# AuburnSounds/audio-formats

Measured on AMD Instinct MI355X. Metric: decoded samples/sec (batched MP3+OGG+FLAC) at 1/2/4/8 MI355X vs CPU ref, higher is better.
Workload: dtype f32 (MP3, Vorbis, CELT) + int32 (FLAC)

## Files before the change

### audio-formats_amd/csrc/mp3_kernel.h

```cpp
#pragma once
#include "afg_common.h"
#ifndef AFG_MP3_FMA
#error "define AFG_MP3_FMA (0 / 1) and AFG_MP3_KERNEL before including mp3_kernel.h"
#endif

#ifndef AFG_MP3_NT_LOAD
#define AFG_MP3_NT_LOAD 0
#endif
#if AFG_MP3_NT_LOAD
typedef float afg_f32x2 __attribute__((ext_vector_type(2)));
#define AFG_MP3_LD(p) ([&] { const afg_f32x2 t_ = __builtin_nontemporal_load((const afg_f32x2 *)(p)); return f2{ t_.x, t_.y }; }())
#else
#define AFG_MP3_LD(p) (*(p))
#endif
#ifndef AFG_MP3_NT_STORE
#define AFG_MP3_NT_STORE 1
#endif

namespace {

struct Mp3Seg {
    uint32_t stream;
    uint32_t g0;
    uint32_t count;
    uint32_t last;
};

struct Mp3Stream {
    uint64_t blk_base;
    uint32_t ngr;
    uint32_t nch;
};

constexpr int kStateOverlap = 64 * 9;

__device__ const float k_aa_cs[8] = {
    0.85749293f, 0.88174200f, 0.94962865f, 0.98331459f, 0.99551782f, 0.99916056f, 0.99989920f, 0.99999316f };
__device__ const float k_aa_ca[8] = {
    0.51449576f, 0.47173197f, 0.31337745f, 0.18191320f, 0.09457419f, 0.04096558f, 0.01419856f, 0.00369997f };

__device__ const float k_win[15 * 16] = {
    -1, 26, -31, 208, 218, 401, -519, 2063, 2000, 4788, -5517, 7134, 5959, 35640, -39336, 74992,
    -1, 24, -35, 202, 222, 347, -581, 2080, 1952, 4425, -5879, 7640, 5288, 33791, -41176, 74856,
    -1, 21, -38, 196, 225, 294, -645, 2087, 1893, 4063, -6237, 8092, 4561, 31947, -43006, 74630,
    -1, 19, -41, 190, 227, 244, -711, 2085, 1822, 3705, -6589, 8492, 3776, 30112, -44821, 74313,
    -1, 17, -45, 183, 228, 197, -779, 2075, 1739, 3351, -6935, 8840, 2935, 28289, -46617, 73908,
    -1, 16, -49, 176, 228, 153, -848, 2057, 1644, 3004, -7271, 9139, 2037, 26482, -48390, 73415,
    -2, 14, -53, 169, 227, 111, -919, 2032, 1535, 2663, -7597, 9389, 1082, 24694, -50137, 72835,
    -2, 13, -58, 161, 224, 72, -991, 2001, 1414, 2330, -7910, 9592, 70, 22929, -51853, 72169,
    -2, 11, -63, 154, 221, 36, -1064, 1962, 1280, 2006, -8209, 9750, -998, 21189, -53534, 71420,
    -2, 10, -68, 147, 215, 2, -1137, 1919, 1131, 1692, -8491, 9863, -2122, 19478, -55178, 70590,
    -3, 9, -73, 139, 208, -29, -1210, 1870, 970, 1388, -8755, 9935, -3300, 17799, -56778, 69679,
    -3, 8, -79, 132, 200, -57, -1283, 1817, 794, 1095, -8998, 9966, -4533, 16155, -58333, 68692,
    -4, 7, -85, 125, 189, -83, -1356, 1759, 605, 814, -9219, 9959, -5818, 14548, -59838, 67629,
    -4, 7, -91, 117, 177, -106, -1428, 1698, 402, 545, -9416, 9916, -7154, 12980, -61289, 66494,
    -5, 6, -97, 111, 163, -127, -1498, 1634, 185, 288, -9585, 9838, -8540, 11455, -62684, 65290 };

__device__ __forceinline__ void dct3_9(float (&y)[9])
{
    float e0 = y[0], e2 = y[2], e4 = y[4], e6 = y[6], e8 = y[8];
    float m0 = e0 + e6 * 0.5f;
    e0 = e0 - e6;
    float m4 = (e4 + e2) * 0.93969262f;
    float m2 = (e8 + e2) * 0.76604444f;
    e6 = (e4 - e8) * 0.17364818f;
    e4 = e4 + (e8 - e2);

    e2 = e0 - e4 * 0.5f;
    y[4] = e4 + e0;
    e8 = m0 - m2 + e6;
    e0 = m0 - m4 + m2;
    e4 = m0 + m4 - e6;

    float o1 = y[1], o3 = y[3], o5 = y[5], o7 = y[7];
    o3 = o3 * 0.86602540f;
    m0 = (o5 + o1) * 0.98480775f;
    m4 = (o5 - o7) * 0.34202014f;
    m2 = (o1 + o7) * 0.64278761f;
    o1 = (o1 - o5 - o7) * 0.86602540f;

    o5 = m0 - o3 - m2;
    o7 = m4 - o3 - m0;
    o3 = m4 + o3 - m2;

    y[0] = e4 - o7;
    y[1] = e2 + o1;
    y[2] = e0 - o3;
    y[3] = e8 + o5;
    y[5] = e8 - o5;
    y[6] = e0 + o3;
    y[7] = e2 - o1;
    y[8] = e4 + o7;
}

__device__ __forceinline__ void imdct36_lane(float (&x)[18], float (&ov)[9], bool stop)
{
    constexpr float tw[18] = {
        0.73727734f, 0.79335334f, 0.84339145f, 0.88701083f, 0.92387953f, 0.95371695f, 0.97629601f, 0.99144486f, 0.99904822f,
        0.67559021f, 0.60876143f, 0.53729961f, 0.46174861f, 0.38268343f, 0.30070580f, 0.21643961f, 0.13052619f, 0.04361938f };
    constexpr float w0[18] = {
        0.99904822f, 0.99144486f, 0.97629601f, 0.95371695f, 0.92387953f, 0.88701083f, 0.84339145f, 0.79335334f, 0.73727734f,
        0.04361938f, 0.13052619f, 0.21643961f, 0.30070580f, 0.38268343f, 0.46174861f, 0.53729961f, 0.60876143f, 0.67559021f };
    constexpr float w1[18] = {
        1, 1, 1, 1, 1, 1, 0.99144486f, 0.92387953f, 0.79335334f,
        0, 0, 0, 0, 0, 0, 0.13052619f, 0.38268343f, 0.60876143f };

    float co[9], si[9];
    co[0] = -x[0];
    si[0] = x[17];
#pragma unroll
    for (int i = 0; i < 4; i++) {
        si[8 - 2 * i] = x[4 * i + 1] - x[4 * i + 2];
        co[1 + 2 * i] = x[4 * i + 1] + x[4 * i + 2];
        si[7 - 2 * i] = x[4 * i + 4] - x[4 * i + 3];
        co[2 + 2 * i] = -(x[4 * i + 3] + x[4 * i + 4]);
    }
    dct3_9(co);
    dct3_9(si);
    si[1] = -si[1];
    si[3] = -si[3];
    si[5] = -si[5];
    si[7] = -si[7];
#pragma unroll
    for (int i = 0; i < 9; i++) {
        float wa = stop ? w1[i] : w0[i];
        float wb = stop ? w1[9 + i] : w0[9 + i];
        float ovl = ov[i];
        float sum = co[i] * tw[9 + i] + si[i] * tw[i];
        ov[i] = co[i] * tw[i] - si[i] * tw[9 + i];
        x[i] = ovl * wa - sum * wb;
        x[17 - i] = ovl * wb + sum * wa;
    }
}

__device__ __forceinline__ void idct3(float x0, float x1, float x2, float (&dst)[3])
{
    float m1 = x1 * 0.86602540f;
    float a1 = x0 - x2 * 0.5f;
    dst[1] = x0 + x2;
    dst[0] = a1 + m1;
    dst[2] = a1 - m1;
}

__device__ __forceinline__ void imdct12(const float (&t)[18], int off, float (&dst)[6], float (&ov)[3])
{
    constexpr float tw3[6] = { 0.79335334f, 0.92387953f, 0.99144486f, 0.60876143f, 0.38268343f, 0.13052619f };
    float co[3], si[3];
    idct3(-t[off + 0], t[off + 6] + t[off + 3], t[off + 12] + t[off + 9], co);
    idct3(t[off + 15], t[off + 12] - t[off + 9], t[off + 6] - t[off + 3], si);
    si[1] = -si[1];
#pragma unroll
    for (int i = 0; i < 3; i++) {
        float ovl = ov[i];
        float sum = co[i] * tw3[3 + i] + si[i] * tw3[i];
        ov[i] = co[i] * tw3[i] - si[i] * tw3[3 + i];
        dst[i] = ovl * tw3[2 - i] - sum * tw3[5 - i];
        dst[5 - i] = ovl * tw3[5 - i] + sum * tw3[2 - i];
    }
}

__device__ __forceinline__ void imdct_short_lane(float (&x)[18], float (&ov)[9])
{
    float t[18];
#pragma unroll
    for (int i = 0; i < 18; i++) t[i] = x[i];
#pragma unroll
    for (int i = 0; i < 6; i++) x[i] = ov[i];
    float tail[3] = { ov[6], ov[7], ov[8] };
    float d[6];
    imdct12(t, 0, d, tail);
#pragma unroll
    for (int i = 0; i < 6; i++) x[6 + i] = d[i];
    imdct12(t, 1, d, tail);
#pragma unroll
    for (int i = 0; i < 6; i++) x[12 + i] = d[i];
    imdct12(t, 2, d, tail);
#pragma unroll
    for (int i = 0; i < 6; i++) ov[i] = d[i];
    ov[6] = tail[0];
    ov[7] = tail[1];
    ov[8] = tail[2];
}

__device__ __forceinline__ void dct2_32(const float (&in)[32], float (&out)[32])
{
    constexpr float sec[24] = {
        10.19000816f, 0.50060302f, 0.50241929f, 3.40760851f, 0.50547093f, 0.52249861f, 2.05778098f, 0.51544732f,
        0.56694406f, 1.48416460f, 0.53104258f, 0.64682180f, 1.16943991f, 0.55310392f, 0.78815460f, 0.97256821f,
        0.58293498f, 1.06067765f, 0.83934963f, 0.62250412f, 1.72244716f, 0.74453628f, 0.67480832f, 5.10114861f };
    float t[4][8];
#pragma unroll
    for (int i = 0; i < 8; i++) {
        float x0 = in[i];
        float x1 = in[15 - i];
        float x2 = in[16 + i];
        float x3 = in[31 - i];
        float t0 = x0 + x3;
        float t1 = x1 + x2;
        float t2 = (x1 - x2) * sec[3 * i + 0];
        float t3 = (x0 - x3) * sec[3 * i + 1];
        t[0][i] = t0 + t1;
        t[1][i] = (t0 - t1) * sec[3 * i + 2];
        t[2][i] = t3 + t2;
        t[3][i] = (t3 - t2) * sec[3 * i + 2];
    }
#pragma unroll
    for (int r = 0; r < 4; r++) {
        float x0 = t[r][0], x1 = t[r][1], x2 = t[r][2], x3 = t[r][3];
        float x4 = t[r][4], x5 = t[r][5], x6 = t[r][6], x7 = t[r][7], xt;
        xt = x0 - x7; x0 = x0 + x7;
        x7 = x1 - x6; x1 = x1 + x6;
        x6 = x2 - x5; x2 = x2 + x5;
        x5 = x3 - x4; x3 = x3 + x4;
        x4 = x0 - x3; x0 = x0 + x3;
        x3 = x1 - x2; x1 = x1 + x2;
        t[r][0] = x0 + x1;
        t[r][4] = (x0 - x1) * 0.70710677f;
        x5 = x5 + x6;
        x6 = (x6 + x7) * 0.70710677f;
        x7 = x7 + xt;
        x3 = (x3 + x4) * 0.70710677f;
        x5 = x5 - x7 * 0.198912367f;
        x7 = x7 + x5 * 0.382683432f;
        x5 = x5 - x7 * 0.198912367f;
        x0 = xt - x6; xt = xt + x6;
        t[r][1] = (xt + x7) * 0.50979561f;
        t[r][2] = (x4 + x3) * 0.54119611f;
        t[r][3] = (x0 - x5) * 0.60134488f;
        t[r][5] = (x0 + x5) * 0.89997619f;
        t[r][6] = (x4 - x3) * 1.30656302f;
        t[r][7] = (xt - x7) * 2.56291556f;
    }
#pragma unroll
    for (int i = 0; i < 7; i++) {
        out[4 * i + 0] = t[0][i];
        out[4 * i + 1] = t[2][i] + t[3][i] + t[3][i + 1];
        out[4 * i + 2] = t[1][i] + t[1][i + 1];
        out[4 * i + 3] = t[2][i + 1] + t[3][i] + t[3][i + 1];
    }
    out[28] = t[0][7];
    out[29] = t[2][7] + t[3][7];
    out[30] = t[1][7];
    out[31] = t[3][7];
}

constexpr int kHS = 66;
constexpr int kHistRows = 15;
constexpr int kRegion = kHistRows * kHS;
constexpr int kLdsFloats = 33 * kHS;
constexpr int kWinStride = 18;

struct alignas(8) f2 { float x, y; };

#define WAVE_SYNC() __builtin_amdgcn_wave_barrier()

__device__ __forceinline__ float from_lane_below(float v)
{
    return __int_as_float(__builtin_amdgcn_update_dpp(0, __float_as_int(v), 0x138, 0xf, 0xf, false));
}
__device__ __forceinline__ float from_lane_above(float v)
{
    return __int_as_float(__builtin_amdgcn_update_dpp(0, __float_as_int(v), 0x130, 0xf, 0xf, false));
}

#ifndef AFG_MP3_MIN_WAVES
#define AFG_MP3_MIN_WAVES 4
#endif

template <int NCH>
__device__ __forceinline__ void mp3_segment(
    const Mp3Seg &seg, const Mp3Stream &st, const float *__restrict__ coef, const uint32_t *__restrict__ flags,
    float *__restrict__ pcm, float *__restrict__ state, float *const H, float *const Wt)
{
    float *const R = H + kRegion;
    const int lane = threadIdx.x;
    constexpr int nch = NCH;
    constexpr int nval = nch * 576;

    const int ch = lane >> 5;
    const int band = lane & 31;
    const int s2 = lane >> 5;
    const int sc = (lane >> 4) & 1;
    const int si = lane & 15;

    const f2 *const wrow = (const f2 *)(Wt + (14 - (si < 15 ? si : 14)) * kWinStride);

    float ov[9];
    const int n_warm = seg.g0 < 2u ? (int)seg.g0 : 2;
    const int g_first = (int)seg.g0 - n_warm;
    const bool from_state = (g_first == 0) && (state != nullptr);
    float *st_blob = state ? state + (size_t)seg.stream * AFG_MP3_STATE_FLOATS : nullptr;
#pragma unroll
    for (int i = 0; i < 9; i++) ov[i] = from_state ? st_blob[lane * 9 + i] : 0.0f;
    for (int r = 0; r < kHistRows; r++)
        H[r * kHS + lane] = from_state ? st_blob[kStateOverlap + r * 64 + lane] : 0.0f;

    const int g_end = (int)(seg.g0 + seg.count);
    const bool ch_on = ch < nch;
    int fbase = g_first;
    uint32_t fl_a = 0, fl_b = 0;
    auto refill = [&](int gb) {
        fbase = gb;
        const int gi = gb + lane;
        fl_a = fl_b = 0;
        if (gi < g_end) {
            fl_a = flags[st.blk_base + (uint64_t)gi * nch];
            if (nch == 2) fl_b = flags[st.blk_base + (uint64_t)gi * nch + 1];
        }
        asm volatile("" : "+v"(fl_a), "+v"(fl_b) : : "memory");
    };
    refill(g_first);
    auto loads_of = [&](int g) -> bool {
        const uint32_t w0 = (uint32_t)__builtin_amdgcn_readlane((int)fl_a, g - fbase);
        const uint32_t w1 = (uint32_t)__builtin_amdgcn_readlane((int)fl_b, g - fbase);
        const uint32_t nz = ((ch ? w1 : w0) >> 24) & 63u;
        return ch_on && band < (int)(nz ? nz - 1u : 32u);
    };
    f2 pre[9];
    {
        const f2 *src = (const f2 *)(coef + (st.blk_base + (uint64_t)g_first * nch) * 576) + lane * 9;
        const bool on = loads_of(g_first);
#pragma unroll
        for (int q = 0; q < 9; q++) pre[q] = f2{ 0.0f, 0.0f };
        if (on) {
#pragma unroll
            for (int q = 0; q < 9; q++) pre[q] = AFG_MP3_LD(src + q);
        }
    }
#pragma unroll
    for (int q = 0; q < 9; q++) asm volatile("" : "+v"(pre[q].x), "+v"(pre[q].y) : : "memory");
    WAVE_SYNC();

    for (int g = g_first; g < g_end; g++) {
        const bool do_synth = g >= (int)seg.g0;
        const bool do_dct = g >= (int)seg.g0 - 1;

        float x[18];
#pragma unroll
        for (int m = 0; m < 9; m++) {
            x[2 * m] = pre[m].x;
            x[2 * m + 1] = pre[m].y;
        }
        if (g + 1 - fbase >= 64) refill(g);
        const uint32_t fl0 = (uint32_t)__builtin_amdgcn_readlane((int)fl_a, g - fbase);
        const uint32_t fl1 = (uint32_t)__builtin_amdgcn_readlane((int)fl_b, g - fbase);
        const uint32_t fl = ch_on ? (ch ? fl1 : fl0) : 0u;
        if (g + 1 < g_end) {
            const f2 *src = (const f2 *)(coef + (st.blk_base + (uint64_t)(g + 1) * nch) * 576) + lane * 9;
            const bool on = loads_of(g + 1);
#pragma unroll
            for (int q = 0; q < 9; q++) pre[q] = f2{ 0.0f, 0.0f };
            if (on) {
#pragma unroll
                for (int q = 0; q < 9; q++) pre[q] = AFG_MP3_LD(src + q);
            }
        }

        if (!(fl0 >> 31)) {
            const int block_type = (int)(fl & 3u);
            const int n_long = (int)((fl >> 8) & 0xffu);
            const int aa = (int)((fl >> 16) & 0xffu) - 1;
            const bool lower = (band >= 1) && (band - 1 < aa);
            const bool upper = (band < aa);
            float nl[8], nh[8];
#pragma unroll
            for (int i = 0; i < 8; i++) {
                float d_prev = from_lane_below(x[17 - i]);
                float u_next = from_lane_above(x[i]);
                nl[i] = x[i] * k_aa_cs[i] - d_prev * k_aa_ca[i];
                nh[i] = u_next * k_aa_ca[i] + x[17 - i] * k_aa_cs[i];
            }
#pragma unroll
            for (int i = 0; i < 8; i++) {
                x[i] = lower ? nl[i] : x[i];
                x[17 - i] = upper ? nh[i] : x[17 - i];
            }
            const bool is_short = (block_type == 2) && (band >= n_long);
            if (is_short) {
                imdct_short_lane(x, ov);
            } else {
                const bool stop = (block_type == 3) && (band >= n_long);
                imdct36_lane(x, ov, stop);
            }
            if (band & 1) {
#pragma unroll
                for (int i = 1; i < 18; i += 2) x[i] = -x[i];
            }
        }

        if (do_dct) {
#pragma unroll
            for (int m = 0; m < 9; m++) ((f2 *)R)[lane * 9 + m] = f2{ x[2 * m], x[2 * m + 1] };
            WAVE_SYNC();

            float out[32];
            const bool dct_lane = (band < 18) && ch_on;
            {
                float in[32];
                const float *col = R + ch * 576 + (dct_lane ? band : 0);
#pragma unroll
                for (int b = 0; b < 32; b++) in[b] = col[b * 18];
                dct2_32(in, out);
            }
            WAVE_SYNC();
            if (dct_lane) {
                f2 *row = (f2 *)(R + band * kHS + ch * 32);
#pragma unroll
                for (int i = 0; i < 15; i++) row[i] = f2{ out[31 - i], out[1 + i] };
                row[15] = f2{ out[16], out[0] };
            }
            WAVE_SYNC();
        }

        if (do_synth) {
            float op0 = 0.0f, op16 = 0.0f;
            const bool pair_lane = (band < 18) && ch_on;
            if (pair_lane) {
                const f2 *base = (const f2 *)(H + band * kHS + ch * 32) + 15;
                f2 z[15];
#pragma unroll
                for (int m = 0; m < 15; m++) z[m] = base[m * (kHS / 2)];
                float a;
                a  = (z[14].x - z[0].x) * 29;
                a += (z[1].x + z[13].x) * 213;
                a += (z[12].x - z[2].x) * 459;
                a += (z[3].x + z[11].x) * 2037;
                a += (z[10].x - z[4].x) * 5153;
                a += (z[5].x + z[9].x) * 6574;
                a += (z[8].x - z[6].x) * 37489;
                a += z[7].x * 75038;
                op0 = a * (1.0f / 32768.0f);
                a  = z[14].y * 104;
                a += z[12].y * 1567;
                a += z[10].y * 9727;
                a += z[8].y * 64019;
                a += z[6].y * -9975;
                a += z[4].y * -45;
                a += z[2].y * 146;
                a += z[0].y * -5;
                op16 = a * (1.0f / 32768.0f);
            }

            f2 w[8];
#pragma unroll
            for (int k = 0; k < 8; k++) w[k] = wrow[k];
            const bool main_lane = (si < 15) && (sc < nch);
            const f2 *base = (const f2 *)(H + s2 * kHS + sc * 32) + (si < 15 ? si : 14);
            const float *rbase = (const float *)base;
            float rw[32];
#pragma unroll
            for (int m = 0; m < 18; m++) rw[m] = rbase[m * kHS + (((m & 1) ^ 0) ? 0 : 1)];
#pragma unroll
            for (int n = 0; n < 9; n++) {
                if (n + 1 < 9 && n > 0) {
                    rw[16 + 2 * n] = rbase[(16 + 2 * n) * kHS + 1];
                    rw[17 + 2 * n] = rbase[(17 + 2 * n) * kHS + 0];
                }
                float a = 0.0f, b = 0.0f;
#pragma unroll
                for (int k = 0; k < 8; k++) {
                    const float vz = rw[15 + 2 * n - k];
                    const float vy = rw[2 * n + k];
#if AFG_MP3_FMA
                    b = __builtin_fmaf(vz, w[k].y, b);
                    b = __builtin_fmaf(vy, w[k].x, b);
                    if (k & 1) {
                        a = __builtin_fmaf(vy, w[k].y, a);
                        a = __builtin_fmaf(-vz, w[k].x, a);
                    } else {
                        a = __builtin_fmaf(vz, w[k].x, a);
                        a = __builtin_fmaf(-vy, w[k].y, a);
                    }
#else
                    const float tb = vz * w[k].y + vy * w[k].x;
                    const float ta = (k & 1) ? (vy * w[k].y - vz * w[k].x) : (vz * w[k].x - vy * w[k].y);
                    b = (k == 0) ? tb : (b + tb);
                    a = (k == 0) ? ta : (a + ta);
#endif
                }
                if (main_lane) {
                    float *pdst = H + ((2 * n + s2) * 32) * nch + sc;
                    pdst[(15 - si) * nch] = a * (1.0f / 32768.0f);
                    pdst[(17 + si) * nch] = b * (1.0f / 32768.0f);
                }
            }
            if (pair_lane) {
                float *pp = H + (band * 32) * nch + ch;
                pp[0] = op0;
                pp[16 * nch] = op16;
            }
            WAVE_SYNC();
#pragma unroll
            for (int q = 0; q < 9; q++) asm volatile("" : "+v"(pre[q].x), "+v"(pre[q].y) : : "memory");
            float4 *dst = (float4 *)(pcm + (st.blk_base + (uint64_t)g * nch) * 576);
#pragma unroll
            for (int q = 0; q < 5; q++) {
                const int idx = lane + 64 * q;
#if AFG_MP3_NT_STORE
                if (4 * idx < nval) {
                    typedef float f32x4nt __attribute__((ext_vector_type(4)));
                    __builtin_nontemporal_store(((const f32x4nt *)H)[idx], (f32x4nt *)dst + idx);
                }
#else
                if (4 * idx < nval) dst[idx] = ((const float4 *)H)[idx];
#endif
            }
        }
        WAVE_SYNC();

        if (do_dct) {
            constexpr int n2 = kHistRows * kHS / 2;
            const f2 *srcp = (const f2 *)(H + 18 * kHS);
            f2 hcp[8];
#pragma unroll
            for (int q = 0; q < 8; q++) {
                const int idx = lane + 64 * q;
                hcp[q] = (idx < n2) ? srcp[idx] : f2{ 0.0f, 0.0f };
            }
#pragma unroll
            for (int q = 0; q < 8; q++) {
                const int idx = lane + 64 * q;
                if (idx < n2) ((f2 *)H)[idx] = hcp[q];
            }
        }
        WAVE_SYNC();
    }

    if (st_blob && seg.last) {
#pragma unroll
        for (int i = 0; i < 9; i++) st_blob[lane * 9 + i] = ov[i];
        for (int r = 0; r < kHistRows; r++) st_blob[kStateOverlap + r * 64 + lane] = H[r * kHS + lane];
    }
}


__global__ __launch_bounds__(64, AFG_MP3_MIN_WAVES) void AFG_MP3_KERNEL(
    const Mp3Seg *__restrict__ segs, const Mp3Stream *__restrict__ streams,
    const float *__restrict__ coef, const uint32_t *__restrict__ flags,
    float *__restrict__ pcm, float *__restrict__ state)
{
    __shared__ __attribute__((aligned(16))) float H[kLdsFloats];
    __shared__ __attribute__((aligned(16))) float Wt[15 * kWinStride];
    const int lane = threadIdx.x;
    for (int i = lane; i < 15 * 16; i += 64) Wt[(i >> 4) * kWinStride + (i & 15)] = k_win[i];
    const Mp3Seg seg = segs[blockIdx.x];
    const Mp3Stream st = streams[seg.stream];
    if (st.nch == 2) mp3_segment<2>(seg, st, coef, flags, pcm, state, H, Wt);
    else mp3_segment<1>(seg, st, coef, flags, pcm, state, H, Wt);
}

}
```

Measured before the change: 795.5 billion.

## Double-buffer MP3 synthesis history in LDS to drop per-granule history copy

```diff
diff --git a/audio-formats_amd/csrc/mp3_kernel.h b/audio-formats_amd/csrc/mp3_kernel.h
--- a/audio-formats_amd/csrc/mp3_kernel.h
+++ b/audio-formats_amd/csrc/mp3_kernel.h
@@ -244,11 +244,19 @@
     out[31] = t[3][7];
 }
 
+#ifndef AFG_MP3_STAGE_PAD
+#define AFG_MP3_STAGE_PAD 1
+#endif
 constexpr int kHS = 66;
 constexpr int kHistRows = 15;
-constexpr int kRegion = kHistRows * kHS;
-constexpr int kLdsFloats = 33 * kHS;
+constexpr int kHalfRows = 18;
+constexpr int kHalf = kHalfRows * kHS;
+constexpr int kHistRow0 = kHalfRows - kHistRows;
+constexpr int kLdsFloats = (2 * kHalfRows + AFG_MP3_STAGE_PAD) * kHS;
+constexpr int kZLen = 3 * kHalfRows;
 constexpr int kWinStride = 18;
+__host__ __device__ constexpr int kStage(int nch) { return 32 * nch + 4 * AFG_MP3_STAGE_PAD; }
+static_assert(17 * kStage(2) + 64 <= kLdsFloats - kHalf, "the staged PCM of a granule leaves the buffer");
 
 struct alignas(8) f2 { float x, y; };
 
@@ -264,15 +272,14 @@
 }
 
 #ifndef AFG_MP3_MIN_WAVES
-#define AFG_MP3_MIN_WAVES 4
+#define AFG_MP3_MIN_WAVES 3
 #endif
 
 template <int NCH>
 __device__ __forceinline__ void mp3_segment(
     const Mp3Seg &seg, const Mp3Stream &st, const float *__restrict__ coef, const uint32_t *__restrict__ flags,
-    float *__restrict__ pcm, float *__restrict__ state, float *const H, float *const Wt)
-{
-    float *const R = H + kRegion;
+    float *__restrict__ pcm, float *__restrict__ state, float *const H, float *const Z, float *const Wt)
+{
     const int lane = threadIdx.x;
     constexpr int nch = NCH;
     constexpr int nval = nch * 576;
@@ -292,8 +299,14 @@
     float *st_blob = state ? state + (size_t)seg.stream * AFG_MP3_STATE_FLOATS : nullptr;
 #pragma unroll
     for (int i = 0; i < 9; i++) ov[i] = from_state ? st_blob[lane * 9 + i] : 0.0f;
-    for (int r = 0; r < kHistRows; r++)
-        H[r * kHS + lane] = from_state ? st_blob[kStateOverlap + r * 64 + lane] : 0.0f;
+    const bool z_lane = (lane & 31) >= 30;
+    float *const zf = Z + ((lane >> 5) * kZLen) * 2 + (lane & 1);
+    for (int r = 0; r < kHistRows; r++) {
+        const float v = from_state ? st_blob[kStateOverlap + r * 64 + lane] : 0.0f;
+        if (z_lane) zf[(kHistRow0 + r) * 2] = v;
+        else H[(kHistRow0 + r) * kHS + lane] = v;
+    }
+    int phase = 0;
 
     const int g_end = (int)(seg.g0 + seg.count);
     const bool ch_on = ch < nch;
@@ -334,6 +347,8 @@
     for (int g = g_first; g < g_end; g++) {
         const bool do_synth = g >= (int)seg.g0;
         const bool do_dct = g >= (int)seg.g0 - 1;
+        const int ob = phase ? kHalf : 0;
+        const int nb = kHalf - ob;
 
         float x[18];
 #pragma unroll
@@ -390,24 +405,30 @@
 
         if (do_dct) {
 #pragma unroll
-            for (int m = 0; m < 9; m++) ((f2 *)R)[lane * 9 + m] = f2{ x[2 * m], x[2 * m + 1] };
+            for (int m = 0; m < 9; m++) ((f2 *)(H + nb))[lane * 9 + m] = f2{ x[2 * m], x[2 * m + 1] };
             WAVE_SYNC();
 
             float out[32];
             const bool dct_lane = (band < 18) && ch_on;
             {
                 float in[32];
-                const float *col = R + ch * 576 + (dct_lane ? band : 0);
+                const float *col = H + nb + ch * 576 + (dct_lane ? band : 0);
 #pragma unroll
                 for (int b = 0; b < 32; b++) in[b] = col[b * 18];
                 dct2_32(in, out);
             }
             WAVE_SYNC();
             if (dct_lane) {
-                f2 *row = (f2 *)(R + band * kHS + ch * 32);
+                f2 *row = (f2 *)(H + nb + band * kHS + ch * 32);
 #pragma unroll
                 for (int i = 0; i < 15; i++) row[i] = f2{ out[31 - i], out[1 + i] };
-                row[15] = f2{ out[16], out[0] };
+                f2 *zrow = (f2 *)Z + ch * kZLen + band;
+                if (phase) {
+                    zrow[0] = f2{ out[16], out[0] };
+                    zrow[2 * kHalfRows] = f2{ out[16], out[0] };
+                } else {
+                    zrow[kHalfRows] = f2{ out[16], out[0] };
+                }
             }
             WAVE_SYNC();
         }
@@ -416,10 +437,10 @@
             float op0 = 0.0f, op16 = 0.0f;
             const bool pair_lane = (band < 18) && ch_on;
             if (pair_lane) {
-                const f2 *base = (const f2 *)(H + band * kHS + ch * 32) + 15;
+                const f2 *base = (const f2 *)Z + ch * kZLen + band + (phase ? kHalfRows + kHistRow0 : kHistRow0);
                 f2 z[15];
 #pragma unroll
-                for (int m = 0; m < 15; m++) z[m] = base[m * (kHS / 2)];
+                for (int m = 0; m < 15; m++) z[m] = base[m];
                 float a;
                 a  = (z[14].x - z[0].x) * 29;
                 a += (z[1].x + z[13].x) * 213;
@@ -445,16 +466,21 @@
 #pragma unroll
             for (int k = 0; k < 8; k++) w[k] = wrow[k];
             const bool main_lane = (si < 15) && (sc < nch);
-            const f2 *base = (const f2 *)(H + s2 * kHS + sc * 32) + (si < 15 ? si : 14);
-            const float *rbase = (const float *)base;
+            const int wcol = sc * 32 + 2 * (si < 15 ? si : 14);
+            const float *rO = H + ob + (kHistRow0 + s2) * kHS + wcol;
+            const float *rN = H + nb + s2 * kHS + wcol;
+            const float *r14 = s2 ? rN - kHS : rO + 14 * kHS;
             float rw[32];
 #pragma unroll
-            for (int m = 0; m < 18; m++) rw[m] = rbase[m * kHS + (((m & 1) ^ 0) ? 0 : 1)];
+            for (int m = 0; m < 14; m++) rw[m] = rO[m * kHS + ((m & 1) ? 0 : 1)];
+            rw[14] = r14[1];
+#pragma unroll
+            for (int m = 15; m < 18; m++) rw[m] = rN[(m - 15) * kHS + ((m & 1) ? 0 : 1)];
 #pragma unroll
             for (int n = 0; n < 9; n++) {
                 if (n + 1 < 9 && n > 0) {
-                    rw[16 + 2 * n] = rbase[(16 + 2 * n) * kHS + 1];
-                    rw[17 + 2 * n] = rbase[(17 + 2 * n) * kHS + 0];
+                    rw[16 + 2 * n] = rN[(1 + 2 * n) * kHS + 1];
+                    rw[17 + 2 * n] = rN[(2 + 2 * n) * kHS + 0];
                 }
                 float a = 0.0f, b = 0.0f;
 #pragma unroll
@@ -479,13 +505,13 @@
 #endif
                 }
                 if (main_lane) {
-                    float *pdst = H + ((2 * n + s2) * 32) * nch + sc;
+                    float *pdst = H + ob + (2 * n + s2) * kStage(nch) + sc;
                     pdst[(15 - si) * nch] = a * (1.0f / 32768.0f);
                     pdst[(17 + si) * nch] = b * (1.0f / 32768.0f);
                 }
             }
             if (pair_lane) {
-                float *pp = H + (band * 32) * nch + ch;
+                float *pp = H + ob + band * kStage(nch) + ch;
                 pp[0] = op0;
                 pp[16 * nch] = op16;
             }
@@ -493,43 +519,34 @@
 #pragma unroll
             for (int q = 0; q < 9; q++) asm volatile("" : "+v"(pre[q].x), "+v"(pre[q].y) : : "memory");
             float4 *dst = (float4 *)(pcm + (st.blk_base + (uint64_t)g * nch) * 576);
+            constexpr int spp = 8 * nch;
+            const float *stg = H + ob + (lane / spp) * kStage(nch) + (lane % spp) * 4;
 #pragma unroll
             for (int q = 0; q < 5; q++) {
                 const int idx = lane + 64 * q;
+                const float *src = stg + q * (64 / spp) * kStage(nch);
 #if AFG_MP3_NT_STORE
                 if (4 * idx < nval) {
                     typedef float f32x4nt __attribute__((ext_vector_type(4)));
-                    __builtin_nontemporal_store(((const f32x4nt *)H)[idx], (f32x4nt *)dst + idx);
+                    __builtin_nontemporal_store(*(const f32x4nt *)src, (f32x4nt *)dst + idx);
                 }
 #else
-                if (4 * idx < nval) dst[idx] = ((const float4 *)H)[idx];
+                if (4 * idx < nval) dst[idx] = *(const float4 *)src;
 #endif
             }
         }
         WAVE_SYNC();
 
-        if (do_dct) {
-            constexpr int n2 = kHistRows * kHS / 2;
-            const f2 *srcp = (const f2 *)(H + 18 * kHS);
-            f2 hcp[8];
-#pragma unroll
-            for (int q = 0; q < 8; q++) {
-                const int idx = lane + 64 * q;
-                hcp[q] = (idx < n2) ? srcp[idx] : f2{ 0.0f, 0.0f };
-            }
-#pragma unroll
-            for (int q = 0; q < 8; q++) {
-                const int idx = lane + 64 * q;
-                if (idx < n2) ((f2 *)H)[idx] = hcp[q];
-            }
-        }
-        WAVE_SYNC();
+        if (do_dct) phase ^= 1;
     }
 
     if (st_blob && seg.last) {
 #pragma unroll
         for (int i = 0; i < 9; i++) st_blob[lane * 9 + i] = ov[i];
-        for (int r = 0; r < kHistRows; r++) st_blob[kStateOverlap + r * 64 + lane] = H[r * kHS + lane];
+        const int ob = phase ? kHalf : 0;
+        for (int r = 0; r < kHistRows; r++)
+            st_blob[kStateOverlap + r * 64 + lane] =
+                z_lane ? zf[((phase ? kHalfRows : 0) + kHistRow0 + r) * 2] : H[ob + (kHistRow0 + r) * kHS + lane];
     }
 }
 
@@ -540,13 +557,14 @@
     float *__restrict__ pcm, float *__restrict__ state)
 {
     __shared__ __attribute__((aligned(16))) float H[kLdsFloats];
+    __shared__ __attribute__((aligned(16))) float Z[2 * kZLen * 2];
     __shared__ __attribute__((aligned(16))) float Wt[15 * kWinStride];
     const int lane = threadIdx.x;
     for (int i = lane; i < 15 * 16; i += 64) Wt[(i >> 4) * kWinStride + (i & 15)] = k_win[i];
     const Mp3Seg seg = segs[blockIdx.x];
     const Mp3Stream st = streams[seg.stream];
-    if (st.nch == 2) mp3_segment<2>(seg, st, coef, flags, pcm, state, H, Wt);
-    else mp3_segment<1>(seg, st, coef, flags, pcm, state, H, Wt);
-}
-
-}
+    if (st.nch == 2) mp3_segment<2>(seg, st, coef, flags, pcm, state, H, Z, Wt);
+    else mp3_segment<1>(seg, st, coef, flags, pcm, state, H, Z, Wt);
+}
+
+}
```

Measured after the change: 795.0 billion. No clear change (-0.1%).
